# WU-CVGL/CasualHDRSplat

Hardware: AMD Instinct MI355X
Metric: train-step images/sec (fwd+bwd raster) @ 1M Gaussians 1080p (higher is better)
Workload: dtype f32; 1 GPU; c3: 1000000 Gaussians, 1920x1080, SH degree 3, HDR radiance + CRF tone-map, 1 pose(s)/view, 1 view(s)/step (one per GPU); num_rendered_R=6777809, R_prime=3025699, pixel_pair_evals_E=559372855, seed=0, binning=sync-free fixed capacity 1.25*R, launch=eager (one enqueue per kernel)

## Files before the change

casualhdrsplat_amd/_lib.py:

```python
from __future__ import annotations

import ctypes as C
import os
import re

_HERE = os.path.dirname(os.path.abspath(__file__))
LIB_PATH = os.environ.get("HS_LIB_PATH", os.path.join(_HERE, "libhdrsplat.so"))

HS_VERSION = 309
HS_OK, HS_EINVAL, HS_EHIP, HS_EOVERFLOW = 0, -1, -2, -3
HS_STAGE_PREPROCESS, HS_STAGE_BIN, HS_STAGE_RENDER, HS_STAGE_ALL, HS_STAGE_OFFSETS = 1, 2, 4, 7, 8
HS_STAGE_PREPROCESS_ONLY = 16
HS_FLAG_HDR, HS_FLAG_BLUR_HDR, HS_FLAG_DEBUG, HS_FLAG_ANTIALIAS = 1, 2, 4, 8
HS_FLAG_RADIANCE_EXP, HS_FLAG_RADIANCE_SOFTPLUS = 16, 32
HS_BWD_RENDER, HS_BWD_PREPROCESS, HS_BWD_CRF, HS_BWD_ALL = 1, 2, 4, 7
HS_BWD_SEGSUM, HS_BWD_PROJECT = 8, 16
HS_TILE = 16
HS_TILE_SORT_RADIX, HS_TILE_SORT_COUNT, HS_TILE_SORT_HIER = 1, 2, 3
HS_DEPTH_SORT_PASSES, HS_DEPTH_SORT_COUNT = 1, 2
HS_CHAIN_BLOCKIDX, HS_CHAIN_TICKETS = 1, 2
HS_EMISSION_SCAN_AHEAD, HS_EMISSION_SCAN_INSIDE = 1, 2

_fp = C.c_void_p

# ... 44 lines not shown
        ("dL_dexposure", _fp), ("dL_dcrf_table", _fp),
        ("dL_dviewmatrices", _fp), ("dL_dprojmatrices", _fp), ("dL_dcamposes", _fp),
        ("dL_dview_colors", _fp), ("dL_dout_invdepth", _fp),
        ("densify_grad_accum", _fp), ("densify_denom", _fp), ("densify_max_radii", _fp),
        ("g_begin", C.c_int32), ("g_end", C.c_int32),
    ]


class hs_layout(C.Structure):
    _fields_ = [(n, C.c_int64) for n in (
        "counters", "rec", "depth", "radii", "tiles_touched", "offsets", "cov3D", "clamped", "scan_spine", "binfo",
        "keys_sorted", "point_list", "pairs_tmp", "ranges", "sort_tmp", "depth_pairs", "inst_sorted", "offs_sorted", "pair_sort_tmp",
        "pair_flags", "pair_act",
        "final_T", "n_contrib", "pose_hdr", "tile_work", "tile_order",
        "pair_grads", "crf_partials", "inst_grads", "pose_partials",
        "tile_matrix", "hier_ws", "depth_ws")]


class hs_loss_args(C.Structure):
    _fields_ = [("planes", C.c_int32), ("H", C.c_int32), ("W", C.c_int32), ("lambda_dssim", C.c_float),
                ("image", _fp), ("target", _fp), ("workspace", _fp), ("partials", _fp), ("out", _fp),
                ("dL_dloss", _fp), ("dL_dimage", _fp)]


HS_ADAM_MAX_GROUPS = 16
HS_ADAM_MASK_NONE, HS_ADAM_MASK_RADII, HS_ADAM_MASK_BYTES = 0, 1, 2


class hs_adam_group(C.Structure):
    _fields_ = [("param", _fp), ("grad", _fp), ("exp_avg", _fp), ("exp_avg_sq", _fp),
                ("rows", C.c_int64), ("row_stride", C.c_int64), ("col_begin", C.c_int64), ("col_count", C.c_int64),
# ... 310 lines not shown
```

casualhdrsplat_amd/csrc/api.hip:

```cpp
#include <stdarg.h>
#include <stdio.h>
#include <stdlib.h>
#include <string.h>
#include <time.h>
#include <unistd.h>
#include <atomic>

#include "hs_cloud.h"

namespace hs {

static thread_local char g_err[512] = "";

#ifdef HS_TESTING
int fault_injection() {
    static const int mode = [] {
        const char* e = getenv("HS_FAULT_INJECT");
        return (e && !strcmp(e, "sort_ticket")) ? 1 : (e && !strcmp(e, "stalled_chain")) ? 2 : (e && !strcmp(e, "late_block")) ? 3 : 0;
    }();
    return mode;
}
#endif

static std::atomic<int> g_sort_tickets{0};
// ... 93 lines not shown
    l.binfo = carve(I * 8);
    sz->geom_bytes = o;
    o = 0;
    l.keys_sorted = carve(2 * align_up(d.capacity * 4, 256));
    l.point_list = l.keys_sorted + align_up(d.capacity * 4, 256);
    l.pairs_tmp = carve(d.capacity * 8);
    l.ranges = carve(vtiles * 8);
    l.sort_tmp = carve(sort_tmp_bytes(I));
    l.depth_ws = carve(depth_ws_words(I) * 4);
    l.depth_pairs = carve(2 * I * 8);
    l.inst_sorted = carve(I * 4);
    l.offs_sorted = carve(I * 4);
    l.pair_sort_tmp = carve(emit_scan_words(I) * 4 + sort_tmp_bytes(d.capacity));
    l.pair_flags = carve(d.capacity);
    l.pair_act = carve(d.capacity);
    l.tile_matrix = carve(count_matrix_words(I, vtiles, d.capacity) * 4);
    l.hier_ws = carve(hier_ws_words(I, gx, gy, d.n_poses, d.capacity) * 4);
    sz->binning_bytes = o;
    o = 0;
    l.final_T = carve(HW * d.n_poses * 4);
    l.n_contrib = carve(HW * d.n_poses * 4);
    l.pose_hdr = carve(HW * 3 * 4 * (d.n_poses + (npf > 1 ? F : 0)));
    l.tile_work = carve(vtiles * 4);
    l.tile_order = carve(vtiles * 4);
    sz->image_bytes = o;
    o = 0;
    l.pair_grads = carve(d.capacity * kPairFloats * 4);
    l.crf_partials = carve(crf_partial_floats(d.crf_K, HW, d.n_poses) * 4);
    l.inst_grads = carve(I * kInstFloats * 4);
    l.pose_partials = carve(pose_partial_floats(d.P, d.n_poses) * 4);
// ... 389 lines not shown
```

casualhdrsplat_amd/csrc/render.hip:

```cpp
#include "hs_common.h"

namespace hs {

namespace {

constexpr float kAlphaMin = 1.0f / 255.0f;
constexpr float kAlphaMax = 0.99f;
constexpr float kTmin = 0.0001f;
constexpr float kLogEps = 1e-8f;


enum {
    kStBwdTrips = 0,
    kStBwdEmpty = 1,
    kStBwdActivePix = 2,
    kStBwdCulled = 3,
    kStBwdHist = 4,
    kStBwdStaged = 10,
    kStBwdBatches = 11,
    kStFwdTrips = 12, kStFwdEmpty = 13, kStFwdActivePix = 14, kStFwdCulled = 15, kStFwdStaged = 16, kStFwdBatches = 17,
    kStCount = 24
};
struct WaveStats {
    unsigned long long v[kStCount];
// ... 83 lines not shown

template <bool TEN>
__device__ __forceinline__ void group_reduce(const float* g, float g9, int xor16_addr, float& t0, float& t1) {
    float w0, w1, w2;
    reduce_in_rows<TEN>(g, g9, w0, w1, w2);
    const float u0 = halve16(w0, w1);
    const float u1 = w2 + __int_as_float(__builtin_amdgcn_ds_bpermute(xor16_addr, __float_as_int(w2)));
    t0 = reduce_in_quads(u0);
    t1 = reduce_in_quads(u1);
}

__device__ __forceinline__ int mask_prefix(uint64_t m) {
    return (int)__builtin_amdgcn_mbcnt_hi((uint32_t)(m >> 32), __builtin_amdgcn_mbcnt_lo((uint32_t)m, 0u));
}

__device__ __forceinline__ uint32_t wave_max_u32(uint32_t v) {
#pragma unroll
    for (int d = 32; d >= 1; d >>= 1) v = max(v, (uint32_t)__shfl_xor((int)v, d));
    return v;
}

struct Crf {
    const float* table;
    int K;
    float umin, umax, dt;
};

__device__ __forceinline__ void crf_locate(const Crf& c, float Hv, int& i, float& f, float& xv, bool& interior) {
    xv = Hv * c.dt;
    const float u = __logf(fmaxf(xv, kLogEps));
    float s = (u - c.umin) / (c.umax - c.umin) * (float)(c.K - 1);
    bool in = true;
    if (!(s > 0.f)) { s = 0.f; in = false; }
    if (s >= (float)(c.K - 1)) { s = (float)(c.K - 1); in = false; }
    i = (int)floorf(s);
    if (i > c.K - 2) i = c.K - 2;
// ... 58 lines not shown
    px = sx + 8 * (lane >> 5) + (lane & 7);
    py0 = sy + 2 * ((lane >> 3) & 3);
}

struct RenderFwd {
    int W, H, gx, ntiles, N, flags;
    const uint2* ranges; const uint32_t* point_list; const float4* rec; const float* bg;
    float* out_color; float* out_hdr; float* final_T; uint32_t* n_contrib; float* pose_hdr;
    float* out_invdepth;
    Crf crf;
    const float* exposure;
    unsigned long long* stats;
    unsigned long long* timeline;
    uint8_t* pair_act;
    uint32_t* tile_work;
};

constexpr int kBatch = 128;

__device__ __forceinline__ int xcd_strip_tile(int b, int nb, int gx) {
    constexpr int kXcd = 8, kRows = 2;
    const int x = b % kXcd, k = b / kXcd;
    const int per = nb / kXcd, rem = nb % kXcd;
    int p = x * per + min(x, rem) + k;
    const int rows = nb / gx;
    const int nstrips = (rows + kRows - 1) / kRows;
    const int strip_tiles = kRows * gx;
    const int last_short = nstrips * strip_tiles - nb;
    int c = 0;
    for (; c < kXcd - 1; ++c) {
// ... 110 lines not shown

    float4 ra = make_float4(0.f, 0.f, 0.f, 0.f), rb = ra;
    float rcb = 0.f, rdepth = 1.f;
    if ((int)threadIdx.x < n) {
        const uint32_t id = p.point_list[range.x + threadIdx.x];
        const float4* r = p.rec + kRecF4 * (int64_t)id;
        ra = r[0]; rb = r[1]; rcb = reinterpret_cast<const float*>(r + 2)[0];
        if constexpr (DEPTH) rdepth = reinterpret_cast<const float*>(r + 2)[1];
    }
    WaveStats ws;
    if constexpr (STATS) ws.clear();
    const char* const ent = reinterpret_cast<const char*>(s_ent);
    float* const my_ent = s_ent + threadIdx.x * kFwdEntF;
    const uint16_t* const my_list = s_list[wave][grp];
    if (threadIdx.x < kFwdEntF) s_ent[KB * kFwdEntF + threadIdx.x] = 0.f;
    auto flush_activity = [&](int base_prev, int cnt_prev) {
        const int t = threadIdx.x;
        if (t < cnt_prev)
            p.pair_act[(int64_t)range.x + base_prev + t] = (uint8_t)(s_taken[0][0][t] | s_taken[0][1][t] | s_taken[1][0][t] | s_taken[1][1][t]);
        s_taken[0][0][t] = 0; s_taken[0][1][t] = 0; s_taken[1][0][t] = 0; s_taken[1][1][t] = 0;
    };
    auto walk = [&](int i0, int i1, int base48) -> uint32_t {
        uint32_t act_lo = 0u, act_hi = 0u;
        uint32_t pos = 0u;
        const uint32_t npos = (uint32_t)(i1 - i0);
        const uint16_t* lp = my_list + i0;
        auto trip = [&]() {
            const int jb = (int)*lp++;
            const char* e = ent + jb;
            const float4 a = *reinterpret_cast<const float4*>(e);
            const float4 b = *reinterpret_cast<const float4*>(e + 16);
            const float2 c = *reinterpret_cast<const float2*>(e + 32);
            const float dx = a.x - pxf;
            const f2 dy = a.y - pyf;
            const float t = a.z * dx * dx, u = a.w * dx;
// ... 12 lines not shown
                "v_writelane_b32 %1, %4, m0\n\t"
                "s_add_u32 %2, %2, 1"
                : "+v"(act_lo), "+v"(act_hi), "+s"(pos) : "s"((uint32_t)took), "s"((uint32_t)(took >> 32)) : "scc", "m0");
#pragma clang diagnostic pop
            if constexpr (STATS) { ws.v[kStFwdTrips] += 1; ws.v[kStFwdEmpty] += took == 0ull; }
        };
        if (npos >= 2u) {
            do {
                trip();
                trip();
            } while (pos + 2u <= npos && (done0 & done1) != ~0ull);
        }
        if (pos + 1u == npos && (done0 & done1) != ~0ull) trip();
        return (act_lo != 0u ? 1u : 0u) | (act_hi != 0u ? 4u : 0u);
    };
    s_taken[0][0][threadIdx.x] = 0; s_taken[0][1][threadIdx.x] = 0; s_taken[1][0][threadIdx.x] = 0; s_taken[1][1][threadIdx.x] = 0;
    uint32_t n_taken = 0;
    int it = 0, base = 0;
    for (; base < n; base += KB, ++it) {
        const uint64_t fin = done0 & done1;
        const bool wave_alive = fin != ~0ull;
        if (lane == 0) s_alive[it & 1][wave] = wave_alive;
        __syncthreads();
        if (it > 0) flush_activity(base - KB, KB);
        if (!(s_alive[it & 1][0] | s_alive[it & 1][1])) break;
        const int cnt = min(KB, n - base);
        if constexpr (STATS) { if (wave == 0) { ws.v[kStFwdStaged] += cnt; ws.v[kStFwdBatches] += 1; } }
        if ((int)threadIdx.x < cnt) {
            scale_entry(ra, rb);
            reinterpret_cast<float4*>(my_ent)[0] = ra;
            reinterpret_cast<float4*>(my_ent)[1] = rb;
            reinterpret_cast<float2*>(my_ent)[4] = make_float2(rcb, DEPTH ? 1.f / rdepth : 0.f);
        }
        if (base + KB + (int)threadIdx.x < n) {
            const uint32_t id = p.point_list[range.x + base + KB + threadIdx.x];
            const float4* r = p.rec + kRecF4 * (int64_t)id;
            ra = r[0]; rb = r[1]; rcb = reinterpret_cast<const float*>(r + 2)[0];
            if constexpr (DEPTH) rdepth = reinterpret_cast<const float*>(r + 2)[1];
        }
        __syncthreads();
        if (wave_alive) {
            const bool alive_g[2] = {(uint32_t)fin != 0xFFFFFFFFu, (uint32_t)(fin >> 32) != 0xFFFFFFFFu};
            int n_g[2] = {0, 0};
#pragma unroll
            for (int k = 0; k < KB / 64; ++k) {
                const int jj = k * 64 + lane;
                bool touch[2] = {false, false};
                if (jj < cnt) {
                    const float4 a = reinterpret_cast<const float4*>(s_ent + jj * kFwdEntF)[0];
                    const float4 b = reinterpret_cast<const float4*>(s_ent + jj * kFwdEntF)[1];
                    touch[0] = alive_g[0] && block_may_touch<8>(a, b, sxf, syf);
                    touch[1] = alive_g[1] && block_may_touch<8>(a, b, sxf + 8.f, syf);
                }
                if constexpr (STATS) ws.v[kStFwdCulled] += __popcll(__ballot(jj < cnt && !touch[0] && !touch[1]));
#pragma unroll
// ... 15 lines not shown
#pragma unroll
            for (int g = 0; g < 2; ++g) {
                const uint32_t bit = 1u << (2 * g);
                if (t0 & bit) s_taken[wave][g][s_list[wave][g][lane] / kEnt] = (uint8_t)(bit << wave);
                if (t1 & bit) s_taken[wave][g][s_list[wave][g][64 + lane] / kEnt] = (uint8_t)(bit << wave);
                n_taken += (uint32_t)(__popcll(__ballot((t0 & bit) != 0u)) + __popcll(__ballot((t1 & bit) != 0u)));
            }
        }
    }
    if (it > 0 && base >= n) {
        __syncthreads();
        flush_activity(base - KB, n - (base - KB));
    }
    if (lane == 0) s_work[wave] = n_taken;
    __syncthreads();
    if (threadIdx.x == 0) p.tile_work[vt] = s_work[0] + s_work[1];
    {
        float* const o = s_ent + wave * (6 * 128);
        const int pos0 = (py0 - sy) * 16 + (px - sx), pos1 = pos0 + 16;
        o[pos0] = ps.T.x; o[pos1] = ps.T.y;
        o[128 + pos0] = __uint_as_float(ps.last0); o[128 + pos1] = __uint_as_float(ps.last1);
        o[256 + pos0] = ps.C0.x; o[256 + pos1] = ps.C0.y;
        o[384 + pos0] = ps.C1.x; o[384 + pos1] = ps.C1.y;
        o[512 + pos0] = ps.C2.x; o[512 + pos1] = ps.C2.y;
        if constexpr (DEPTH) { o[640 + pos0] = ps.D.x; o[640 + pos1] = ps.D.y; }
        const int qx = sx + (lane & 15), qy0 = sy + 2 * (lane >> 4);
        const int r0 = (qy0 - sy) * 16 + (lane & 15), r1 = r0 + 16;
        PixF s0, s1;
        s0.T = o[r0]; s0.last = __float_as_uint(o[128 + r0]) / (kFwdEntF * 4); s0.C0 = o[256 + r0]; s0.C1 = o[384 + r0]; s0.C2 = o[512 + r0];
        s1.T = o[r1]; s1.last = __float_as_uint(o[128 + r1]) / (kFwdEntF * 4); s1.C0 = o[256 + r1]; s1.C1 = o[384 + r1]; s1.C2 = o[512 + r1];
        const bool q0 = qx < p.W && qy0 < p.H, q1 = qx < p.W && qy0 + 1 < p.H;
// ... 207 lines not shown
            if (k == 0) v += NW == 4 ? ((s_wave[0][1] + s_wave[1][1]) + s_wave[2 % NW][1]) + s_wave[3 % NW][1] : s_wave[0][1] + s_wave[1][1];
            if (k == K - 1) v += NW == 4 ? ((s_wave[0][2] + s_wave[1][2]) + s_wave[2 % NW][2]) + s_wave[3 % NW][2] : s_wave[0][2] + s_wave[1][2];
        }
        dst[k] = v;
    }
}

struct RenderBwd {
    int W, H, gx, gy, ntiles, N, F, flags;
    const uint2* ranges; const uint32_t* point_list; const float4* rec; const float* bg;
    const float* final_T; const uint32_t* n_contrib; const float* pose_hdr;
    const float* dL_dcolor; const float* dL_dhdr; const float* dL_dalpha; const float* dL_dinvdepth;
    float4* pair_grads;
    uint8_t* pair_flags;
    const uint8_t* pair_act;
    Crf crf;
    const float* exposure;
    unsigned long long* stats;
    unsigned long long* timeline;
    uint32_t* queue;
    const uint32_t* tile_order;
    int grid_tiles;
    CrfGradArgs crf_tail;
};

__device__ __forceinline__ float pixel_grad(const RenderBwd& p, const Crf& c, int pose, int frame, int ch, int64_t pix, int64_t HW) {
    const float invN = 1.f / (float)p.N;
    const int64_t gpl = ((int64_t)frame * 3 + ch) * HW + pix;
    float g = p.dL_dcolor[gpl];
    if (!(p.flags & HS_FLAG_HDR)) return g * invN;
// ... 51 lines not shown
    const f2 ae = {act0 ? alpha.x : 0.f, act1 ? alpha.y : 0.f};
    const f2 one_m = splat(1.f) - ae;
    const f2 rcp = {__builtin_amdgcn_rcpf(one_m.x), __builtin_amdgcn_rcpf(one_m.y)};
    s.T *= rcp;
    dch = ae * s.T;
    f2 cd = (splat(r) * s.dL0 + pk_mul_hi(f2{r, g}, s.dL1)) + splat(b) * s.dL2;
    if constexpr (DEPTH) cd += splat(invd) * s.dLd;
    const f2 diff = cd - s.q;
    const f2 gd = G * (diff * s.T);
    s.q += ae * diff;
    dop = f2{act0 ? gd.x : 0.f, act1 ? gd.y : 0.f};
    sw = splat(o) * dop;
}

constexpr int kTailPct = 8;
constexpr int kAccF = 12;
constexpr int kBwdKB = 52;


template <bool DEPTH, bool STATS>
__global__ void __launch_bounds__(kBatch) __attribute__((amdgpu_waves_per_eu((DEPTH || STATS) ? 1 : 7)))
render_bwd_kernel(RenderBwd p) {
    constexpr int KB = kBwdKB;
    constexpr int NV = DEPTH ? 10 : 9;
    constexpr int kEntF = kAccF + 4 * NV;
    constexpr int kEntB = kEntF * 4;
    static_assert(kEntB % 16 == 0, "LDS entry records must stay 16-byte aligned");
    constexpr int kSentinel = KB * kEntB;
    constexpr int kListLen = KB + 8;
    __shared__ __attribute__((aligned(16))) float s_ent[(KB + 1) * kEntF];
    static_assert(KB * kEntF >= 2 * 7 * 128, "the pixel-state re-deal of the prologue borrows the staging area below the sentinel");
    __shared__ uint16_t s_list[2][2][kListLen];
    __shared__ uint8_t s_actb[kBatch];
    __shared__ uint32_t s_max[2];

    __shared__ uint32_t s_q;
    if constexpr (!STATS) {
        if ((int)blockIdx.x >= p.grid_tiles) {
            const int qd = (int)blockIdx.x - p.grid_tiles;
            crf_grad_body<2>(p.crf_tail, qd % p.crf_tail.bx, qd / p.crf_tail.bx, reinterpret_cast<unsigned long long*>(s_ent));
            return;
        }
    }
    const int n_tail = (int)((int64_t)p.grid_tiles * kTailPct / 100);
    const int n_static = p.grid_tiles - n_tail;
    if (threadIdx.x < kAccF) s_ent[KB * kEntF + threadIdx.x] = 0.f;
    for (;;) {
    int bidx = blockIdx.x;
    if ((int)blockIdx.x >= n_static) {
        __syncthreads();
        if (threadIdx.x == 0) {
            const uint32_t q = atomicAdd(p.queue, 1u);
            if (q == 2u * (uint32_t)n_tail - 1u) atomicExch(p.queue, 0u);
            s_q = q;
        }
        __syncthreads();
        if (s_q >= (uint32_t)n_tail) return;
        bidx = n_static + (int)s_q;
    }
    const int vt = p.tile_order ? (int)p.tile_order[bidx] : xcd_strip_tile(bidx, p.grid_tiles, p.gx);
    const int pose = vt / p.ntiles;
    const int tile = vt - pose * p.ntiles;
    const int tx = tile % p.gx, ty = tile / p.gx;
    const int wave = threadIdx.x >> 6, lane = threadIdx.x & 63;
    const int grp = lane >> 5;
    const int sx = tx * kTile, sy = ty * kTile + wave * 8;
    int px, py0;
    lane_pixels(lane, sx, sy, px, py0);
    const int py1 = py0 + 1;
    const float pxf = (float)px;
    const f2 pyf = {(float)py0, (float)py1};

    unsigned long long t_start = 0;
    if constexpr (STATS) t_start = wall_clock64();
    const uint2 range = p.ranges[vt];

    PixB s0, s1;
    {
        const int qx = sx + (lane & 15), qy0 = sy + 2 * (lane >> 4);
        PixB t0, t1;
        const int frame = p.F > 1 ? pose / p.N : 0;
        load_pixel_bwd(p, t0, qx < p.W && qy0 < p.H, pose, frame, qx, qy0);
        load_pixel_bwd(p, t1, qx < p.W && qy0 + 1 < p.H, pose, frame, qx, qy0 + 1);
        float* const o = s_ent + wave * (7 * 128);
        const int r0 = (qy0 - sy) * 16 + (lane & 15), r1 = r0 + 16;
        o[r0] = t0.T; o[r1] = t1.T;
        o[128 + r0] = t0.dL0; o[128 + r1] = t1.dL0;
        o[256 + r0] = t0.dL1; o[256 + r1] = t1.dL1;
        o[384 + r0] = t0.dL2; o[384 + r1] = t1.dL2;
        o[512 + r0] = t0.q; o[512 + r1] = t1.q;
        o[640 + r0] = t0.dLd; o[640 + r1] = t1.dLd;
        o[768 + r0] = __uint_as_float(t0.last); o[768 + r1] = __uint_as_float(t1.last);
        __builtin_amdgcn_fence(__ATOMIC_RELEASE, "wavefront");
        __builtin_amdgcn_wave_barrier();
        const int p0 = (py0 - sy) * 16 + (px - sx), p1 = p0 + 16;
        s0.T = o[p0]; s0.dL0 = o[128 + p0]; s0.dL1 = o[256 + p0]; s0.dL2 = o[384 + p0]; s0.q = o[512 + p0];
        s0.dLd = o[640 + p0]; s0.last = __float_as_uint(o[768 + p0]);
        s1.T = o[p1]; s1.dL0 = o[128 + p1]; s1.dL1 = o[256 + p1]; s1.dL2 = o[384 + p1]; s1.q = o[512 + p1];
        s1.dLd = o[640 + p1]; s1.last = __float_as_uint(o[768 + p1]);
    }
    PairB ps = pack_pair(s0, s1);

    const uint32_t wave_max = wave_max_u32(max(s0.last, s1.last));
    if (lane == 0) s_max[wave] = wave_max;
    __syncthreads();
    const int n_proc = (int)max(s_max[0], s_max[1]);

    int red_off = -1;
    const bool red_t0 = (lane & 3) == 0;
    {
        const int row = lane >> 4, k = (lane & 15) >> 2;
        constexpr int kOrd[4] = {0, 2, 1, 3};
        if ((lane & 3) == 0) red_off = ((row & 1) ? 4 : 0) + kOrd[k];
        else if ((lane & 3) == 1 && !(row & 1) && k == 0) red_off = 8;
        else if (DEPTH && (lane & 3) == 1 && !(row & 1) && k == 2) red_off = 9;
        if (red_off >= 0) red_off = (kAccF + NV * (2 * grp + wave) + red_off) * 4;
    }
    const int xor16_addr = (lane ^ 16) << 2;
    char* const ent = reinterpret_cast<char*>(s_ent);
    float* const my_ent = s_ent + threadIdx.x * kEntF;
    const uint16_t* const my_list = s_list[wave][grp];
    WaveStats ws;
    if constexpr (STATS) ws.clear();
    const int nb = (n_proc + KB - 1) / KB;
    uint32_t id_next = 0, act_next = 0;
    if (nb > 0) {
        const int base = (nb - 1) * KB;
        if ((int)threadIdx.x < n_proc - base) {
            id_next = p.point_list[range.x + base + threadIdx.x];
            act_next = p.pair_act[(int64_t)range.x + base + threadIdx.x];
        }
    }
    for (int bi = nb - 1; bi >= 0; --bi) {
        const int base = bi * KB;
        const int cnt = min(KB, n_proc - base);
        if constexpr (STATS) { if (wave == 0) { ws.v[kStBwdStaged] += cnt; ws.v[kStBwdBatches] += 1; } }
        __syncthreads();
        const bool taken = (int)threadIdx.x < cnt && act_next != 0;
        s_actb[threadIdx.x] = (uint8_t)((int)threadIdx.x < cnt ? act_next : 0u);
        if (taken) {
            const float4* r = p.rec + kRecF4 * (int64_t)id_next;
            float4 ra = r[0], rb = r[1];
            float4 rc = r[2];
            if constexpr (DEPTH) rc.y = 1.f / rc.y;
            scale_entry(ra, rb);
            reinterpret_cast<float4*>(my_ent)[0] = ra;
            reinterpret_cast<float4*>(my_ent)[1] = rb;
            reinterpret_cast<float4*>(my_ent)[2] = rc;
        }
        if (bi > 0 && (int)threadIdx.x < KB) {
            id_next = p.point_list[range.x + base - KB + threadIdx.x];
            act_next = p.pair_act[(int64_t)range.x + base - KB + threadIdx.x];
        }
        __syncthreads();
        {
            int maxn = 0;
#pragma unroll
            for (int g = 0; g < 2; ++g) {
                const uint32_t gbit = 1u << (2 * g + wave);
                uint16_t* lst = s_list[wave][g];
                int n_g = 0;
#pragma unroll
                for (int k = (KB + 63) / 64 - 1; k >= 0; --k) {
                    const uint64_t m = __ballot((s_actb[k * 64 + lane] & gbit) != 0);
                    const int c = __popcll(m);
                    if ((m >> lane) & 1ull) lst[n_g + c - 1 - mask_prefix(m)] = (uint16_t)((k * 64 + lane) * kEntB);
                    n_g += c;
                }
#pragma unroll
                for (int t = lane; t < kListLen; t += 64)
                    if (t >= n_g) lst[t] = (uint16_t)kSentinel;
                maxn = max(maxn, n_g);
            }
            if constexpr (STATS) {
                const uint32_t wbits = 5u << wave;
                uint32_t mine = 0;
#pragma unroll
                for (int k = 0; k < (KB + 63) / 64; ++k) mine += __popcll(__ballot((s_actb[k * 64 + lane] & wbits) != 0));
                ws.v[kStBwdCulled] += (uint32_t)cnt - mine;
            }
            const int lim0 = ((int)s0.last - base) * kEntB, lim1 = ((int)s1.last - base) * kEntB;
            int jb = (int)my_list[0];
            for (int ti = 0; ti < maxn; ++ti) {
                int jn = (int)my_list[ti + 1];
                asm("" : "+v"(jn));
                const float4 a = *reinterpret_cast<const float4*>(ent + jb);
                const float4 b = *reinterpret_cast<const float4*>(ent + jb + 16);
                const float2 c = *reinterpret_cast<const float2*>(ent + jb + 32);
                const float cb = c.x;
                const float invd = DEPTH ? c.y : 0.f;
                const float dx = a.x - pxf;
                const f2 dy = a.y - pyf;
                const float t = a.z * dx * dx, u = a.w * dx;
                const f2 pw = dy * (b.x * dy + u) + t;
                const float G0 = hs_exp2(pw.x), G1 = hs_exp2(pw.y);
                const float al0 = fminf(kAlphaMax, b.y * G0), al1 = fminf(kAlphaMax, b.y * G1);
                const bool act0 = (jb < lim0) && (pw.x <= 0.f) && (al0 >= kAlphaMin);
                const bool act1 = (jb < lim1) && (pw.y <= 0.f) && (al1 >= kAlphaMin);
                if constexpr (STATS) {
                    const int lanes = __popcll(__ballot(act0 || act1));
                    ws.v[kStBwdTrips] += 1;
                    ws.v[kStBwdEmpty] += lanes == 0;
                    ws.v[kStBwdActivePix] += __popcll(__ballot(act0)) + __popcll(__ballot(act1));
                    const int bin = lanes == 0 ? 0 : lanes <= 4 ? 1 : lanes <= 8 ? 2 : lanes <= 16 ? 3 : lanes <= 32 ? 4 : 5;
                    ws.v[kStBwdHist + bin] += 1;
                }
                f2 sw, dop, dch;
                step_bwd_pair<DEPTH>(ps, act0, act1, f2{G0, G1}, f2{al0, al1}, b.y, b.z, b.w, cb, invd, sw, dop, dch);
                const f2 m = sw * dy;
                const f2 m2 = m * dy;
                const f2 c0 = dch * ps.dL0, c1 = dch * ps.dL1, c2 = dch * ps.dL2;
                float g[9];
                g[0] = (sw.x + sw.y) * dx;
                g[1] = m.x + m.y;
                g[2] = g[0] * dx;
                g[3] = g[1] * dx;
                g[4] = m2.x + m2.y;
                g[5] = dop.x + dop.y;
                g[6] = c0.x + c0.y;
                g[7] = c1.x + c1.y;
                g[8] = c2.x + c2.y;
                float g9 = 0.f;
                if constexpr (DEPTH) {
                    const f2 cd = dch * ps.dLd;
                    g9 = cd.x + cd.y;
                }
                float t0, t1;
                group_reduce<DEPTH>(g, g9, xor16_addr, t0, t1);
                if (red_off >= 0) *reinterpret_cast<float*>(ent + jb + red_off) = red_t0 ? t0 : t1;
                jb = jn;
            }
        }
        __syncthreads();
        if (taken) {
            float v[10] = {0.f, 0.f, 0.f, 0.f, 0.f, 0.f, 0.f, 0.f, 0.f, 0.f};
            const uint32_t ab = s_actb[threadIdx.x];
#pragma unroll
            for (int pl = 0; pl < 4; ++pl) {
                const bool on = (ab >> pl) & 1u;
#pragma unroll
                for (int q = 0; q < NV; ++q) {
                    const float x = my_ent[kAccF + NV * pl + q];
                    v[q] += on ? x : 0.f;
                }
            }
            const float4 a = reinterpret_cast<const float4*>(my_ent)[0];
            const float4 c = reinterpret_cast<const float4*>(my_ent)[2];
            const float A = a.z * (-2.f / kLog2e), B = a.w * (-1.f / kLog2e), C = my_ent[4] * (-2.f / kLog2e);
            const float ddelx_dx = 0.5f * (float)p.W, ddely_dy = 0.5f * (float)p.H;
            const float gmx = -(A * v[0] + B * v[1]) * ddelx_dx;
            const float gmy = -(C * v[1] + B * v[0]) * ddely_dy;
            const int rad = __float_as_int(c.z);
            const uint32_t off = __float_as_uint(c.w);
            const int rminx = min(p.gx, max(0, (int)((a.x - (float)rad) / (float)kTile)));
            const int rminy = min(p.gy, max(0, (int)((a.y - (float)rad) / (float)kTile)));
            const int rmaxx = min(p.gx, max(0, (int)((a.x + (float)rad + (float)(kTile - 1)) / (float)kTile)));
            const int64_t slot = (int64_t)off + (int64_t)(ty - rminy) * (rmaxx - rminx) + (tx - rminx);
            p.pair_flags[slot] = 1;
            float4* o = p.pair_grads + kPairF4 * slot;
            o[0] = make_float4(gmx, gmy, -0.5f * v[2], -v[3]);
            o[1] = make_float4(-0.5f * v[4], v[5], v[6], v[7]);
            o[2] = make_float4(v[8], v[9], 0.f, 0.f);
            if constexpr (kPairF4 == 4) o[3] = make_float4(0.f, 0.f, 0.f, 0.f);
        }
    }
    if constexpr (STATS) {
        ws.flush(p.stats);
        if (p.timeline && threadIdx.x == 0) {
            p.timeline[3 * bidx + 0] = t_start;
            p.timeline[3 * bidx + 1] = wall_clock64();
            const uint32_t xcc = __builtin_amdgcn_s_getreg((3 << 11) | (0 << 6) | 20);
            const uint32_t hw = __builtin_amdgcn_s_getreg((31 << 11) | (0 << 6) | 4);
            p.timeline[3 * bidx + 2] = ((unsigned long long)xcc << 32) | hw;
        }
    }
    if ((int)blockIdx.x < n_static) return;
    }
}

__global__ void __launch_bounds__(256) crf_grad_kernel(CrfGradArgs A) {
    extern __shared__ unsigned long long s_crf_tab[];
    crf_grad_body<4>(A, (int)blockIdx.x, (int)blockIdx.y, s_crf_tab);
}
// ... 13 lines not shown
    const int F = frames_of(d);
    p.ntiles = p.gx * gy; p.N = d.n_poses / F; p.flags = a.flags;
    char* bin = (char*)a.binning; char* img = (char*)a.image; char* geom = (char*)a.geom;
    p.ranges = (const uint2*)(bin + L.ranges); p.point_list = (const uint32_t*)(bin + L.point_list);
    p.rec = (const float4*)(geom + L.rec); p.bg = a.bg;
    p.out_color = a.out_color; p.out_hdr = a.out_hdr;
    p.final_T = (float*)(img + L.final_T); p.n_contrib = (uint32_t*)(img + L.n_contrib);
    const bool need_pose = (a.flags & HS_FLAG_HDR) || p.N > 1;
    p.pose_hdr = need_pose ? (float*)(img + L.pose_hdr) : nullptr;
    p.crf.table = a.crf_table; p.crf.K = a.crf_K; p.crf.umin = a.crf_umin; p.crf.umax = a.crf_umax; p.crf.dt = 1.f;
    p.exposure = a.exposure;
    p.out_invdepth = a.out_invdepth;
    p.stats = stats; p.timeline = nullptr;
    p.pair_act = (uint8_t*)bin + L.pair_act;
    p.tile_work = (uint32_t*)(img + L.tile_work);
    const int grid = p.ntiles * d.n_poses;
    if (stats) {
        if (a.out_invdepth) render_fwd_kernel<true, true><<<grid, kBatch, 0, s>>>(p);
        else render_fwd_kernel<false, true><<<grid, kBatch, 0, s>>>(p);
    } else if (a.out_invdepth) render_fwd_kernel<true, false><<<grid, kBatch, 0, s>>>(p);
    else render_fwd_kernel<false, false><<<grid, kBatch, 0, s>>>(p);
    HS_LAUNCH_CHECK();
    if (orders_tiles(grid)) {
        const int n_static = grid - (int)((int64_t)grid * kTailPct / 100);
        order_tiles_kernel<<<8, 1024, 0, s>>>(grid, p.gx, n_static, p.tile_work, (uint32_t*)(img + L.tile_order));
        HS_LAUNCH_CHECK();
    }
    if (p.N > 1) {
        const int64_t HW = (int64_t)d.W * d.H;
        resolve_kernel<<<ceil_div((int64_t)F * 3 * HW, 256), 256, 0, s>>>(HW, p.N, F, a.flags, p.pose_hdr, p.crf, a.exposure,
// ... 39 lines not shown
    p.W = d.W; p.H = d.H; p.gx = (d.W + kTile - 1) / kTile; p.gy = (d.H + kTile - 1) / kTile;
    p.F = frames_of(d);
    p.ntiles = p.gx * p.gy; p.N = d.n_poses / p.F; p.flags = a.flags;
    const char* bin = (const char*)a.binning; const char* img = (const char*)a.image; const char* geom = (const char*)a.geom;
    p.ranges = (const uint2*)(bin + L.ranges); p.point_list = (const uint32_t*)(bin + L.point_list);
    p.rec = (const float4*)(geom + L.rec); p.bg = a.bg;
    p.final_T = (const float*)(img + L.final_T); p.n_contrib = (const uint32_t*)(img + L.n_contrib);
    p.pose_hdr = (const float*)(img + L.pose_hdr);
    p.dL_dcolor = a.dL_dout_color; p.dL_dhdr = a.dL_dout_hdr; p.dL_dalpha = a.dL_dout_alpha;
    p.dL_dinvdepth = a.dL_dout_invdepth;
    p.pair_grads = (float4*)((char*)a.bwd + L.pair_grads);
    p.crf.table = a.crf_table; p.crf.K = a.crf_K; p.crf.umin = a.crf_umin; p.crf.umax = a.crf_umax; p.crf.dt = 1.f;
    p.exposure = a.exposure;
    p.pair_flags = (uint8_t*)a.binning + L.pair_flags;
    p.pair_act = (const uint8_t*)a.binning + L.pair_act;
    p.stats = stats; p.timeline = timeline;
    p.queue = &((hs_counters*)((char*)a.geom + L.counters))->reserved[3];
    p.tile_order = orders_tiles(p.ntiles * d.n_poses) ? (const uint32_t*)(img + L.tile_order) : nullptr;
    int grid = p.ntiles * d.n_poses;
    p.grid_tiles = grid;
    if (crf_in_tail && !stats && crf_grad_args(a, L, p.crf_tail, 2)) grid += p.crf_tail.bx * p.crf_tail.planes;
    if (stats) {
        if (a.dL_dout_invdepth) render_bwd_kernel<true, true><<<grid, kBatch, 0, s>>>(p);
        else render_bwd_kernel<false, true><<<grid, kBatch, 0, s>>>(p);
    } else if (a.dL_dout_invdepth) render_bwd_kernel<true, false><<<grid, kBatch, 0, s>>>(p);
    else render_bwd_kernel<false, false><<<grid, kBatch, 0, s>>>(p);
    HS_LAUNCH_CHECK();
    return HS_OK;
}

// ... 8 lines not shown
```

include/hdrsplat.h:

```cpp
#ifndef HDRSPLAT_H
#define HDRSPLAT_H

#include <stdint.h>

#ifdef __cplusplus
extern "C" {
#endif

#define HS_API __attribute__((visibility("default")))

#define HS_VERSION 309

#define HS_OK 0
#define HS_EINVAL (-1)
#define HS_EHIP (-2)
#define HS_EOVERFLOW (-3)

#define HS_TILE 16

#define HS_STAGE_PREPROCESS 1
#define HS_STAGE_BIN 2
#define HS_STAGE_RENDER 4
#define HS_STAGE_ALL 7
#define HS_STAGE_OFFSETS 8
// ... 131 lines not shown
    int32_t* densify_max_radii;
    int32_t g_begin, g_end;
} hs_bwd_args;

typedef struct hs_layout {
    int64_t counters, rec, depth, radii, tiles_touched, offsets, cov3D, clamped, scan_spine, binfo;
    int64_t keys_sorted, point_list, pairs_tmp, ranges, sort_tmp, depth_pairs, inst_sorted, offs_sorted, pair_sort_tmp;
    int64_t pair_flags;
    int64_t pair_act;
    int64_t final_T, n_contrib, pose_hdr;
    int64_t tile_work, tile_order;
    int64_t pair_grads, crf_partials, inst_grads, pose_partials;
    int64_t tile_matrix;
    int64_t hier_ws;
    int64_t depth_ws;
} hs_layout;

HS_API int hs_version(void);
HS_API const char* hs_last_error(void);
HS_API int hs_plan(const hs_dims* dims, hs_sizes* sizes, hs_layout* layout );
HS_API int hs_forward(const hs_fwd_args* args, void* hip_stream);
HS_API int hs_backward(const hs_bwd_args* args, void* hip_stream);
HS_API int hs_max_frames(void);
HS_API int hs_mark_visible(int32_t P, const float* means3D, const float* viewmatrix, uint8_t* visible,
                    void* hip_stream);

HS_API int hs_sh_backward_views(int32_t P, int32_t M, int32_t sh_degree, int32_t V, const float* means3D,
                         const float* camposes , const float* dL_dview_colors ,
                         float* dL_dshs , void* hip_stream);

// ... 449 lines not shown
```

Before: 963.5 images/s.

## Compact active pair list in forward and restructure backward staging around it

The forward render now writes a compacted per-tile list of pair indices that touched any pixel, along with a count per tile. The backward kernel walks this compacted list instead of every pair up to the max last-contributor. This removes staging and evaluation of culled pairs, and also drops the wave-max reduction and its extra barrier. Gradient sums move out of the entry records into a separate LDS region addressed by per-group slot numbers. Batches whose per-group active count exceeds L are split, and a wave-split mode lets one wave stage the next batch while the other writes results. The cost is an extra global write and read of the index list, plus more LDS and control logic.

```diff
diff --git a/casualhdrsplat_amd/_lib.py b/casualhdrsplat_amd/_lib.py
--- a/casualhdrsplat_amd/_lib.py
+++ b/casualhdrsplat_amd/_lib.py
@@ -82,7 +82,7 @@
         "pair_flags", "pair_act",
         "final_T", "n_contrib", "pose_hdr", "tile_work", "tile_order",
         "pair_grads", "crf_partials", "inst_grads", "pose_partials",
-        "tile_matrix", "hier_ws", "depth_ws")]
+        "tile_matrix", "hier_ws", "depth_ws", "pair_taken", "tile_taken")]
 
 
 class hs_loss_args(C.Structure):
diff --git a/casualhdrsplat_amd/csrc/api.hip b/casualhdrsplat_amd/csrc/api.hip
--- a/casualhdrsplat_amd/csrc/api.hip
+++ b/casualhdrsplat_amd/csrc/api.hip
@@ -131,6 +131,8 @@
     l.pair_sort_tmp = carve(emit_scan_words(I) * 4 + sort_tmp_bytes(d.capacity));
     l.pair_flags = carve(d.capacity);
     l.pair_act = carve(d.capacity);
+    l.pair_taken = carve(d.capacity * 4);
+    l.tile_taken = carve(vtiles * 4);
     l.tile_matrix = carve(count_matrix_words(I, vtiles, d.capacity) * 4);
     l.hier_ws = carve(hier_ws_words(I, gx, gy, d.n_poses, d.capacity) * 4);
     sz->binning_bytes = o;
diff --git a/casualhdrsplat_amd/csrc/render.hip b/casualhdrsplat_amd/csrc/render.hip
--- a/casualhdrsplat_amd/csrc/render.hip
+++ b/casualhdrsplat_amd/csrc/render.hip
@@ -121,12 +121,6 @@
     return (int)__builtin_amdgcn_mbcnt_hi((uint32_t)(m >> 32), __builtin_amdgcn_mbcnt_lo((uint32_t)m, 0u));
 }
 
-__device__ __forceinline__ uint32_t wave_max_u32(uint32_t v) {
-#pragma unroll
-    for (int d = 32; d >= 1; d >>= 1) v = max(v, (uint32_t)__shfl_xor((int)v, d));
-    return v;
-}
-
 struct Crf {
     const float* table;
     int K;
@@ -215,6 +209,8 @@
     unsigned long long* timeline;
     uint8_t* pair_act;
     uint32_t* tile_work;
+    uint32_t* pair_taken;
+    uint32_t* tile_taken;
 };
 
 constexpr int kBatch = 128;
@@ -355,11 +351,17 @@
     float* const my_ent = s_ent + threadIdx.x * kFwdEntF;
     const uint16_t* const my_list = s_list[wave][grp];
     if (threadIdx.x < kFwdEntF) s_ent[KB * kFwdEntF + threadIdx.x] = 0.f;
+    uint32_t n_list = 0;
     auto flush_activity = [&](int base_prev, int cnt_prev) {
-        const int t = threadIdx.x;
-        if (t < cnt_prev)
-            p.pair_act[(int64_t)range.x + base_prev + t] = (uint8_t)(s_taken[0][0][t] | s_taken[0][1][t] | s_taken[1][0][t] | s_taken[1][1][t]);
-        s_taken[0][0][t] = 0; s_taken[0][1][t] = 0; s_taken[1][0][t] = 0; s_taken[1][1][t] = 0;
+        const int t = threadIdx.x, u = t ^ 64;
+        const uint32_t mine = s_taken[0][0][t] | s_taken[0][1][t] | s_taken[1][0][t] | s_taken[1][1][t];
+        const uint32_t other = s_taken[0][0][u] | s_taken[0][1][u] | s_taken[1][0][u] | s_taken[1][1][u];
+        if (t < cnt_prev) p.pair_act[(int64_t)range.x + base_prev + t] = (uint8_t)mine;
+        const bool on = t < cnt_prev && mine != 0u;
+        const uint64_t m = __ballot(on), mu = __ballot(u < cnt_prev && other != 0u);
+        const uint32_t lead = wave ? (uint32_t)__popcll(mu) : 0u;
+        if (on) p.pair_taken[(int64_t)range.x + n_list + lead + (uint32_t)mask_prefix(m)] = (uint32_t)(base_prev + t);
+        n_list += (uint32_t)(__popcll(m) + __popcll(mu));
     };
     auto walk = [&](int i0, int i1, int base48) -> uint32_t {
         uint32_t act_lo = 0u, act_hi = 0u;
@@ -402,7 +404,6 @@
         if (pos + 1u == npos && (done0 & done1) != ~0ull) trip();
         return (act_lo != 0u ? 1u : 0u) | (act_hi != 0u ? 4u : 0u);
     };
-    s_taken[0][0][threadIdx.x] = 0; s_taken[0][1][threadIdx.x] = 0; s_taken[1][0][threadIdx.x] = 0; s_taken[1][1][threadIdx.x] = 0;
     uint32_t n_taken = 0;
     int it = 0, base = 0;
     for (; base < n; base += KB, ++it) {
@@ -427,6 +428,8 @@
             if constexpr (DEPTH) rdepth = reinterpret_cast<const float*>(r + 2)[1];
         }
         __syncthreads();
+        s_taken[wave][0][lane] = 0; s_taken[wave][0][64 + lane] = 0;
+        s_taken[wave][1][lane] = 0; s_taken[wave][1][64 + lane] = 0;
         if (wave_alive) {
             const bool alive_g[2] = {(uint32_t)fin != 0xFFFFFFFFu, (uint32_t)(fin >> 32) != 0xFFFFFFFFu};
             int n_g[2] = {0, 0};
@@ -472,7 +475,7 @@
     }
     if (lane == 0) s_work[wave] = n_taken;
     __syncthreads();
-    if (threadIdx.x == 0) p.tile_work[vt] = s_work[0] + s_work[1];
+    if (threadIdx.x == 0) { p.tile_work[vt] = s_work[0] + s_work[1]; p.tile_taken[vt] = n_list; }
     {
         float* const o = s_ent + wave * (6 * 128);
         const int pos0 = (py0 - sy) * 16 + (px - sx), pos1 = pos0 + 16;
@@ -710,6 +713,8 @@
     float4* pair_grads;
     uint8_t* pair_flags;
     const uint8_t* pair_act;
+    const uint32_t* pair_taken;
+    const uint32_t* tile_taken;
     Crf crf;
     const float* exposure;
     unsigned long long* stats;
@@ -791,42 +796,61 @@
 }
 
 constexpr int kTailPct = 8;
-constexpr int kAccF = 12;
-constexpr int kBwdKB = 52;
+#ifndef HS_TUNE_BWD_KB
+#define HS_TUNE_BWD_KB 64
+#endif
+#ifndef HS_TUNE_BWD_L
+#define HS_TUNE_BWD_L 50
+#endif
+#ifndef HS_TUNE_BWD_SPLIT
+#define HS_TUNE_BWD_SPLIT 1
+#endif
+constexpr int kBwdKB = HS_TUNE_BWD_KB;
+constexpr int kBwdL = HS_TUNE_BWD_L;
+static_assert(kBwdKB <= kBatch && kBwdL >= 1 && kBwdL < kBwdKB && kBwdL <= 255, "batch <= workgroup, slot numbers fit a byte");
 
 
 template <bool DEPTH, bool STATS>
 __global__ void __launch_bounds__(kBatch) __attribute__((amdgpu_waves_per_eu((DEPTH || STATS) ? 1 : 7)))
 render_bwd_kernel(RenderBwd p) {
     constexpr int KB = kBwdKB;
+    constexpr int L = kBwdL;
+    constexpr int kR = (KB + 63) / 64;
     constexpr int NV = DEPTH ? 10 : 9;
-    constexpr int kEntF = kAccF + 4 * NV;
+    constexpr int kEntF = DEPTH ? 16 : 12;
+    constexpr int kIdxB = DEPTH ? 48 : 36;
     constexpr int kEntB = kEntF * 4;
     static_assert(kEntB % 16 == 0, "LDS entry records must stay 16-byte aligned");
+    constexpr int kSumF = 4 * L * NV;
+    static_assert(kSumF % 4 == 0, "the records behind the sums must stay 16-byte aligned");
     constexpr int kSentinel = KB * kEntB;
-    constexpr int kListLen = KB + 8;
-    __shared__ __attribute__((aligned(16))) float s_ent[(KB + 1) * kEntF];
-    static_assert(KB * kEntF >= 2 * 7 * 128, "the pixel-state re-deal of the prologue borrows the staging area below the sentinel");
+    constexpr int kListLen = (L + 2 + 1) & ~1;
+    __shared__ __attribute__((aligned(16))) float s_mem[kSumF + (KB + 1) * kEntF];
+    static_assert(kSumF + KB * kEntF >= 2 * 7 * 128, "the pixel-state re-deal of the prologue borrows the area below the sentinel");
+    static_assert(kSumF + (KB + 1) * kEntF >= 2 * 1023, "the CRF tail keeps its table of up to 1023 64-bit words here");
+    float* const s_sum = s_mem;
+    float* const s_ent = s_mem + kSumF;
     __shared__ uint16_t s_list[2][2][kListLen];
     __shared__ uint8_t s_actb[kBatch];
-    __shared__ uint32_t s_max[2];
+    __shared__ __attribute__((aligned(4))) uint8_t s_pos[KB][4];
 
     __shared__ uint32_t s_q;
     if constexpr (!STATS) {
         if ((int)blockIdx.x >= p.grid_tiles) {
             const int qd = (int)blockIdx.x - p.grid_tiles;
-            crf_grad_body<2>(p.crf_tail, qd % p.crf_tail.bx, qd / p.crf_tail.bx, reinterpret_cast<unsigned long long*>(s_ent));
+            crf_grad_body<2>(p.crf_tail, qd % p.crf_tail.bx, qd / p.crf_tail.bx, reinterpret_cast<unsigned long long*>(s_mem));
             return;
         }
     }
     const int n_tail = (int)((int64_t)p.grid_tiles * kTailPct / 100);
     const int n_static = p.grid_tiles - n_tail;
-    if (threadIdx.x < kAccF) s_ent[KB * kEntF + threadIdx.x] = 0.f;
+    if (threadIdx.x < kEntF) s_ent[KB * kEntF + threadIdx.x] = 0.f;
+    const int wave = __builtin_amdgcn_readfirstlane((int)(threadIdx.x >> 6));
     for (;;) {
     int bidx = blockIdx.x;
     if ((int)blockIdx.x >= n_static) {
         __syncthreads();
-        if (threadIdx.x == 0) {
+        if (__builtin_amdgcn_mbcnt_lo(~0u, 0u) == 0u && wave == 0) {
             const uint32_t q = atomicAdd(p.queue, 1u);
             if (q == 2u * (uint32_t)n_tail - 1u) atomicExch(p.queue, 0u);
             s_q = q;
@@ -839,7 +863,8 @@
     const int pose = vt / p.ntiles;
     const int tile = vt - pose * p.ntiles;
     const int tx = tile % p.gx, ty = tile / p.gx;
-    const int wave = threadIdx.x >> 6, lane = threadIdx.x & 63;
+    int lane;
+    asm volatile("v_mbcnt_lo_u32_b32 %0, -1, 0\n\tv_mbcnt_hi_u32_b32 %0, -1, %0" : "=v"(lane));
     const int grp = lane >> 5;
     const int sx = tx * kTile, sy = ty * kTile + wave * 8;
     int px, py0;
@@ -851,6 +876,33 @@
     unsigned long long t_start = 0;
     if constexpr (STATS) t_start = wall_clock64();
     const uint2 range = p.ranges[vt];
+    const int n_list = (int)p.tile_taken[vt];
+
+    const bool wave1 = wave != 0;
+    constexpr bool kSplit = HS_TUNE_BWD_SPLIT && KB <= 64;
+    const int e = kSplit ? lane : 64 * wave + lane;
+    int hi = n_list;
+    const bool stager = !kSplit || wave1, writer = !kSplit || !wave1;
+    uint32_t idx_next = 0, id_next = 0;
+    auto prefetch = [&](int hi_n) {
+        const int lo_n = max(0, hi_n - KB);
+        if (stager && e < hi_n - lo_n) {
+            idx_next = p.pair_taken[(int64_t)range.x + lo_n + e];
+            id_next = p.point_list[(int64_t)range.x + idx_next];
+        }
+    };
+    float4 ra = make_float4(0.f, 0.f, 0.f, 0.f), rb = ra, rc = ra;
+    uint32_t act = 0, idx_r = 0;
+    auto gather = [&](int hi_n) {
+        act = 0; idx_r = 0;
+        ra = make_float4(0.f, 0.f, 0.f, 0.f); rb = ra; rc = ra;
+        if (stager && e < min(KB, hi_n)) {
+            const float4* r = p.rec + kRecF4 * (int64_t)id_next;
+            ra = r[0]; rb = r[1]; rc = r[2];
+            act = p.pair_act[(int64_t)range.x + idx_next];
+            idx_r = idx_next;
+        }
+    };
 
     PixB s0, s1;
     {
@@ -859,7 +911,7 @@
         const int frame = p.F > 1 ? pose / p.N : 0;
         load_pixel_bwd(p, t0, qx < p.W && qy0 < p.H, pose, frame, qx, qy0);
         load_pixel_bwd(p, t1, qx < p.W && qy0 + 1 < p.H, pose, frame, qx, qy0 + 1);
-        float* const o = s_ent + wave * (7 * 128);
+        float* const o = s_mem + wave * (7 * 128);
         const int r0 = (qy0 - sy) * 16 + (lane & 15), r1 = r0 + 16;
         o[r0] = t0.T; o[r1] = t1.T;
         o[128 + r0] = t0.dL0; o[128 + r1] = t1.dL0;
@@ -878,11 +930,6 @@
     }
     PairB ps = pack_pair(s0, s1);
 
-    const uint32_t wave_max = wave_max_u32(max(s0.last, s1.last));
-    if (lane == 0) s_max[wave] = wave_max;
-    __syncthreads();
-    const int n_proc = (int)max(s_max[0], s_max[1]);
-
     int red_off = -1;
     const bool red_t0 = (lane & 3) == 0;
     {
@@ -891,72 +938,104 @@
         if ((lane & 3) == 0) red_off = ((row & 1) ? 4 : 0) + kOrd[k];
         else if ((lane & 3) == 1 && !(row & 1) && k == 0) red_off = 8;
         else if (DEPTH && (lane & 3) == 1 && !(row & 1) && k == 2) red_off = 9;
-        if (red_off >= 0) red_off = (kAccF + NV * (2 * grp + wave) + red_off) * 4;
-    }
+    }
+    float* const my_sum = s_sum + (2 * grp + wave) * (L * NV) + max(red_off, 0);
     const int xor16_addr = (lane ^ 16) << 2;
     char* const ent = reinterpret_cast<char*>(s_ent);
-    float* const my_ent = s_ent + threadIdx.x * kEntF;
+    float* const my_ent = s_ent + (e < KB ? e : KB) * kEntF;
     const uint16_t* const my_list = s_list[wave][grp];
     WaveStats ws;
     if constexpr (STATS) ws.clear();
-    const int nb = (n_proc + KB - 1) / KB;
-    uint32_t id_next = 0, act_next = 0;
-    if (nb > 0) {
-        const int base = (nb - 1) * KB;
-        if ((int)threadIdx.x < n_proc - base) {
-            id_next = p.point_list[range.x + base + threadIdx.x];
-            act_next = p.pair_act[(int64_t)range.x + base + threadIdx.x];
-        }
-    }
-    for (int bi = nb - 1; bi >= 0; --bi) {
-        const int base = bi * KB;
-        const int cnt = min(KB, n_proc - base);
-        if constexpr (STATS) { if (wave == 0) { ws.v[kStBwdStaged] += cnt; ws.v[kStBwdBatches] += 1; } }
+    prefetch(hi);
+    if constexpr (kSplit) gather(hi);
+    while (hi > 0) {
+        const int lo = max(0, hi - KB);
+        const int cnt = hi - lo;
         __syncthreads();
-        const bool taken = (int)threadIdx.x < cnt && act_next != 0;
-        s_actb[threadIdx.x] = (uint8_t)((int)threadIdx.x < cnt ? act_next : 0u);
-        if (taken) {
-            const float4* r = p.rec + kRecF4 * (int64_t)id_next;
-            float4 ra = r[0], rb = r[1];
-            float4 rc = r[2];
-            if constexpr (DEPTH) rc.y = 1.f / rc.y;
-            scale_entry(ra, rb);
-            reinterpret_cast<float4*>(my_ent)[0] = ra;
-            reinterpret_cast<float4*>(my_ent)[1] = rb;
-            reinterpret_cast<float4*>(my_ent)[2] = rc;
-        }
-        if (bi > 0 && (int)threadIdx.x < KB) {
-            id_next = p.point_list[range.x + base - KB + threadIdx.x];
-            act_next = p.pair_act[(int64_t)range.x + base - KB + threadIdx.x];
-        }
+        if constexpr (!kSplit) gather(hi);
+        if (stager) {
+            if (e < cnt) {
+                scale_entry(ra, rb);
+                if constexpr (DEPTH) {
+                    rc.y = 1.f / rc.y;
+                    my_ent[12] = __uint_as_float(idx_r);
+                } else {
+                    rc.y = __uint_as_float(idx_r);
+                }
+                reinterpret_cast<float4*>(my_ent)[0] = ra;
+                reinterpret_cast<float4*>(my_ent)[1] = rb;
+                reinterpret_cast<float4*>(my_ent)[2] = rc;
+            }
+            s_actb[e] = (uint8_t)act;
+        }
+        prefetch(lo);
         __syncthreads();
+        int j0 = 0;
         {
+            uint64_t mg[2][kR];
+            int most = 0;
+#pragma unroll
+            for (int g = 0; g < 2; ++g) {
+                int c0 = 0, c1 = 0;
+#pragma unroll
+                for (int k = 0; k < kR; ++k) {
+                    const uint32_t ab = s_actb[k * 64 + lane];
+                    const uint64_t m0 = __ballot((ab >> (2 * g)) & 1u), m1 = __ballot((ab >> (2 * g + 1)) & 1u);
+                    c0 += __popcll(m0); c1 += __popcll(m1);
+                    mg[g][k] = wave1 ? m1 : m0;
+                }
+                most = max(most, max(c0, c1));
+            }
+            if (most > L) {
+                do {
+                    ++j0;
+                    most = 0;
+#pragma unroll
+                    for (int b = 0; b < 4; ++b) {
+                        int c = 0;
+#pragma unroll
+                        for (int k = 0; k < kR; ++k)
+                            c += __popcll(__ballot(k * 64 + lane >= j0 && ((s_actb[k * 64 + lane] >> b) & 1u)));
+                        most = max(most, c);
+                    }
+                } while (most > L);
+#pragma unroll
+                for (int g = 0; g < 2; ++g)
+#pragma unroll
+                    for (int k = 0; k < kR; ++k)
+                        mg[g][k] &= j0 <= k * 64 ? ~0ull : (j0 >= k * 64 + 64 ? 0ull : ~0ull << (j0 - k * 64));
+            }
+            if constexpr (STATS) {
+                if (wave == 0) { ws.v[kStBwdStaged] += cnt - j0; ws.v[kStBwdBatches] += 1; }
+                uint32_t both = 0;
+#pragma unroll
+                for (int k = 0; k < kR; ++k) both += __popcll(mg[0][k] | mg[1][k]);
+                ws.v[kStBwdCulled] += (uint32_t)(cnt - j0) - both;
+            }
             int maxn = 0;
 #pragma unroll
             for (int g = 0; g < 2; ++g) {
-                const uint32_t gbit = 1u << (2 * g + wave);
                 uint16_t* lst = s_list[wave][g];
                 int n_g = 0;
 #pragma unroll
-                for (int k = (KB + 63) / 64 - 1; k >= 0; --k) {
-                    const uint64_t m = __ballot((s_actb[k * 64 + lane] & gbit) != 0);
-                    const int c = __popcll(m);
-                    if ((m >> lane) & 1ull) lst[n_g + c - 1 - mask_prefix(m)] = (uint16_t)((k * 64 + lane) * kEntB);
+                for (int k = kR - 1; k >= 0; --k) {
+                    const uint64_t mk = mg[g][k];
+                    const int c = __popcll(mk);
+                    if ((mk >> lane) & 1ull) {
+                        const int slot = n_g + c - 1 - mask_prefix(mk);
+                        lst[slot] = (uint16_t)((k * 64 + lane) * kEntB);
+                        s_pos[k * 64 + lane][2 * g + wave] = (uint8_t)slot;
+                    }
                     n_g += c;
                 }
 #pragma unroll
-                for (int t = lane; t < kListLen; t += 64)
-                    if (t >= n_g) lst[t] = (uint16_t)kSentinel;
+                for (int k = 0; k < (kListLen + 63) / 64; ++k) {
+                    const int t = k * 64 + lane;
+                    if (t >= n_g && t < kListLen) lst[t] = (uint16_t)kSentinel;
+                }
                 maxn = max(maxn, n_g);
             }
-            if constexpr (STATS) {
-                const uint32_t wbits = 5u << wave;
-                uint32_t mine = 0;
-#pragma unroll
-                for (int k = 0; k < (KB + 63) / 64; ++k) mine += __popcll(__ballot((s_actb[k * 64 + lane] & wbits) != 0));
-                ws.v[kStBwdCulled] += (uint32_t)cnt - mine;
-            }
-            const int lim0 = ((int)s0.last - base) * kEntB, lim1 = ((int)s1.last - base) * kEntB;
+            const uint32_t last0 = s0.last, last1 = s1.last;
             int jb = (int)my_list[0];
             for (int ti = 0; ti < maxn; ++ti) {
                 int jn = (int)my_list[ti + 1];
@@ -966,14 +1045,15 @@
                 const float2 c = *reinterpret_cast<const float2*>(ent + jb + 32);
                 const float cb = c.x;
                 const float invd = DEPTH ? c.y : 0.f;
+                const uint32_t idx = DEPTH ? *reinterpret_cast<const uint32_t*>(ent + jb + kIdxB) : __float_as_uint(c.y);
                 const float dx = a.x - pxf;
                 const f2 dy = a.y - pyf;
                 const float t = a.z * dx * dx, u = a.w * dx;
                 const f2 pw = dy * (b.x * dy + u) + t;
                 const float G0 = hs_exp2(pw.x), G1 = hs_exp2(pw.y);
                 const float al0 = fminf(kAlphaMax, b.y * G0), al1 = fminf(kAlphaMax, b.y * G1);
-                const bool act0 = (jb < lim0) && (pw.x <= 0.f) && (al0 >= kAlphaMin);
-                const bool act1 = (jb < lim1) && (pw.y <= 0.f) && (al1 >= kAlphaMin);
+                const bool act0 = (idx < last0) && (pw.x <= 0.f) && (al0 >= kAlphaMin);
+                const bool act1 = (idx < last1) && (pw.y <= 0.f) && (al1 >= kAlphaMin);
                 if constexpr (STATS) {
                     const int lanes = __popcll(__ballot(act0 || act1));
                     ws.v[kStBwdTrips] += 1;
@@ -1004,21 +1084,21 @@
                 }
                 float t0, t1;
                 group_reduce<DEPTH>(g, g9, xor16_addr, t0, t1);
-                if (red_off >= 0) *reinterpret_cast<float*>(ent + jb + red_off) = red_t0 ? t0 : t1;
+                if (red_off >= 0) my_sum[ti * NV] = red_t0 ? t0 : t1;
                 jb = jn;
             }
         }
         __syncthreads();
-        if (taken) {
+        if (writer && e < cnt && e >= j0) {
             float v[10] = {0.f, 0.f, 0.f, 0.f, 0.f, 0.f, 0.f, 0.f, 0.f, 0.f};
-            const uint32_t ab = s_actb[threadIdx.x];
+            const uint32_t ab = s_actb[e];
+            const uint32_t pos4 = *reinterpret_cast<const uint32_t*>(s_pos[e]);
 #pragma unroll
             for (int pl = 0; pl < 4; ++pl) {
-                const bool on = (ab >> pl) & 1u;
-#pragma unroll
-                for (int q = 0; q < NV; ++q) {
-                    const float x = my_ent[kAccF + NV * pl + q];
-                    v[q] += on ? x : 0.f;
+                if ((ab >> pl) & 1u) {
+                    const float* const sp = s_sum + (pl * L + (int)((pos4 >> (8 * pl)) & 255u)) * NV;
+#pragma unroll
+                    for (int q = 0; q < NV; ++q) v[q] += sp[q];
                 }
             }
             const float4 a = reinterpret_cast<const float4*>(my_ent)[0];
@@ -1037,13 +1117,22 @@
             float4* o = p.pair_grads + kPairF4 * slot;
             o[0] = make_float4(gmx, gmy, -0.5f * v[2], -v[3]);
             o[1] = make_float4(-0.5f * v[4], v[5], v[6], v[7]);
-            o[2] = make_float4(v[8], v[9], 0.f, 0.f);
-            if constexpr (kPairF4 == 4) o[3] = make_float4(0.f, 0.f, 0.f, 0.f);
-        }
+            float z = 0.f;
+            asm volatile("" : "+v"(z));
+            o[2] = make_float4(v[8], v[9], z, z);
+            if constexpr (kPairF4 == 4) o[3] = make_float4(z, z, z, z);
+        }
+        if (j0 > 0) {
+            hi = lo + j0;
+            prefetch(hi);
+        } else {
+            hi = lo;
+        }
+        if constexpr (kSplit) gather(hi);
     }
     if constexpr (STATS) {
         ws.flush(p.stats);
-        if (p.timeline && threadIdx.x == 0) {
+        if (p.timeline && lane == 0 && wave == 0) {
             p.timeline[3 * bidx + 0] = t_start;
             p.timeline[3 * bidx + 1] = wall_clock64();
             const uint32_t xcc = __builtin_amdgcn_s_getreg((3 << 11) | (0 << 6) | 20);
@@ -1087,6 +1176,8 @@
     p.stats = stats; p.timeline = nullptr;
     p.pair_act = (uint8_t*)bin + L.pair_act;
     p.tile_work = (uint32_t*)(img + L.tile_work);
+    p.pair_taken = (uint32_t*)(bin + L.pair_taken);
+    p.tile_taken = (uint32_t*)(bin + L.tile_taken);
     const int grid = p.ntiles * d.n_poses;
     if (stats) {
         if (a.out_invdepth) render_fwd_kernel<true, true><<<grid, kBatch, 0, s>>>(p);
@@ -1156,6 +1247,8 @@
     p.exposure = a.exposure;
     p.pair_flags = (uint8_t*)a.binning + L.pair_flags;
     p.pair_act = (const uint8_t*)a.binning + L.pair_act;
+    p.pair_taken = (const uint32_t*)(bin + L.pair_taken);
+    p.tile_taken = (const uint32_t*)(bin + L.tile_taken);
     p.stats = stats; p.timeline = timeline;
     p.queue = &((hs_counters*)((char*)a.geom + L.counters))->reserved[3];
     p.tile_order = orders_tiles(p.ntiles * d.n_poses) ? (const uint32_t*)(img + L.tile_order) : nullptr;
diff --git a/include/hdrsplat.h b/include/hdrsplat.h
--- a/include/hdrsplat.h
+++ b/include/hdrsplat.h
@@ -169,6 +169,7 @@
     int64_t tile_matrix;
     int64_t hier_ws;
     int64_t depth_ws;
+    int64_t pair_taken, tile_taken;
 } hs_layout;
 
 HS_API int hs_version(void);
```

New measurement: 972.0 images/s, median of 3. No clear change (+0.9%).
